# CIS565-Fall-2015/Project3-CUDA-Path-Tracer

Hardware: AMD Instinct MI355X
Metric: Mpaths/sec (paths = pixels x bounces x spp) at 1280x720, 8 bounces (higher is better)
Workload: dtype f32; 1 GPU; scenes/cornell.txt 1280x720, 8 bounces, 64 spp per step x 149 steps; batches_in_flight=3

## Files before the change

### project3-cuda-path-tracer_amd/__init__.py

```python
import ctypes as C
import os

import numpy as np

HERE = os.path.dirname(os.path.abspath(__file__))
LIB_PATH = os.environ.get("PT_AMD_LIB") or os.path.join(HERE, "csrc", "libpt_amd.so")
HOST_LIB_PATH = os.path.join(HERE, "host", "libpt_host.so")

GEOM_DTYPE = np.dtype([
    ("type", "<i4"), ("materialid", "<i4"),
    ("translation", "<f4", 3), ("rotation", "<f4", 3), ("scale", "<f4", 3),
    ("transform", "<f4", 16), ("inverseTransform", "<f4", 16), ("invTranspose", "<f4", 16),
])
MATERIAL_DTYPE = np.dtype([
    ("color", "<f4", 3), ("specularExponent", "<f4"), ("specularColor", "<f4", 3),
    ("hasReflective", "<f4"), ("hasRefractive", "<f4"), ("indexOfRefraction", "<f4"),
    ("emittance", "<f4"),
])
CAMERA_DTYPE = np.dtype([
    ("resolution", "<i4", 2), ("position", "<f4", 3), ("view", "<f4", 3), ("up", "<f4", 3),
    ("fov", "<f4", 2),
])
assert GEOM_DTYPE.itemsize == 236 and MATERIAL_DTYPE.itemsize == 44 and CAMERA_DTYPE.itemsize == 52

# ... 39 lines not shown
    "pt_test_bump_normal", "pt_test_denoise", "pt_test_denoise_var", "pt_test_noise_stats", "pt_test_exp_neg_poly", "pt_test_bounce_form", "pt_test_live_device_buffers",
    "pt_test_renderer_state", "pt_test_scene_plan", "pt_test_temporal", "pt_test_temporal_camera", "pt_test_history",
    "pt_test_display", "pt_test_spatial_variance",
    "pt_test_group_create_virtual", "pt_test_emulated_reduce",
]


class PtOptions(C.Structure):
    _fields_ = [("shard_rank", C.c_int32), ("shard_count", C.c_int32), ("device", C.c_int32),
                ("flags", C.c_int32), ("pipeline_depth", C.c_int32), ("max_batch", C.c_int32),
                ("stream", C.c_void_p), ("accum_dev", C.c_void_p), ("lens_radius", C.c_float), ("focal_distance", C.c_float)]


class PtTestPlanSummary(C.Structure):
    _fields_ = [("state_bits", C.c_uint32)] + [(n, C.c_int32) for n in ("nBinned", "nWalls", "nSphCull", "nSphGroups", "nLocalPad", "firstSkipped", "poolChunks")] + \
               [("ldsBytes", C.c_uint64), ("ldsBytesNext", C.c_uint64)]


class PtMesh(C.Structure):
    _fields_ = [("geom", C.c_int32), ("ntris", C.c_int32), ("tris", C.c_void_p), ("normals", C.c_void_p), ("materials", C.c_void_p)]


class PtTexture(C.Structure):
    _fields_ = [("width", C.c_int32), ("height", C.c_int32), ("rgb", C.c_void_p)]


class PtTexBinding(C.Structure):
    _fields_ = [("geom", C.c_int32), ("texture", C.c_int32), ("ntris", C.c_int32), ("uvs", C.c_void_p)]


class PtBumpBinding(C.Structure):
# ... 1123 lines not shown
```

### project3-cuda-path-tracer_amd/csrc/pt_api.hip

```cpp
#include <hip/hip_runtime.h>

#include <algorithm>
#include <array>
#include <atomic>
#include <condition_variable>
#include <functional>
#include <thread>
#include <cmath>
#include <cstdarg>
#include <cstdio>
#include <cstdlib>
#include <cstring>
#include <deque>
#include <limits>
#include <map>
#include <memory>
#include <string>
#include <utility>
#include <vector>

#include <mutex>

#include "../../include/pt_amd.h"
#include "pt_compaction.h"
// ... 284 lines not shown
    const PathPool out = pool(sl, depth & 1);
    const uint32_t genIn = sl.gen[(depth - 1) & 1];
    if (++R().launchSerial == 0u) ++R().launchSerial;
    const uint32_t genOut = sl.gen[depth & 1] = R().launchSerial;
    hipEvent_t e0 = nullptr, e1 = nullptr;
    if (R().flags & PT_FLAG_KERNEL_TIMING) {
        for (hipEvent_t *e : {&e0, &e1}) {
            if (!R().evFree.empty()) { *e = R().evFree.back(); R().evFree.pop_back(); }
            else HIPCHECK(hipEventCreate(e));
        }
        HIPCHECK(hipEventRecord(e0, sl.stream));
    }
    BounceArgs ba;
    ba.prm = R().prm;
    ba.iter = iter; ba.batch = batch; ba.depth = depth; ba.lastBounce = lastBounce ? 1 : 0; ba.parity = sl.parity;
    ba.genIn = genIn; ba.genOut = genOut;
    ba.in = in; ba.out = out;
    ba.tile.inBase = in.base; ba.tile.inList = in.list; ba.tile.inCap = in.cap;
    ba.tile.genIn = genIn; ba.tile.poolChunks = (uint32_t)R().prm.poolChunks; ba.tile.chunkShift = (uint32_t)R().prm.chunkShift;
    ba.tile.skipNonCandidates = (lastBounce && R().prm.emittersBinned) ? 1u : 0u;
    ba.tile.hot = (lastBounce ? kHotLast : 0u) | (R().prm.allClassified ? kHotAllClassified : 0u) | (contrib ? kHotContrib : 0u) |
                  ((R().prm.directDepth != 0 && depth == R().prm.directDepth && R().prm.nEmit > 0) ? kHotToLight : 0u) |
                  (R().prm.contribLocal ? kHotContribLocal : 0u) | ((R().flags & PT_FLAG_MIXTURE_WEIGHTED) ? kHotMixWeighted : 0u) | ((uint32_t)R().prm.nWalls << 8) | ((uint32_t)R().prm.nSlotWalls << 11) | ((uint32_t)R().prm.nPlaneWalls << 17) |
                  ((uint32_t)R().prm.nBinned << 14) | ((uint32_t)R().prm.nmats << 20);
    const bool lastBits = R().many && !R().mesh && R().prm.sphOMax > 0.0f && R().prm.emittersBinned;
    if (lastBits && nextIsLast) ba.tile.hot |= kHotWritesLastBits;
    if (lastBits && lastBounce && depth > 1) ba.tile.hot |= kHotReadsLastBits;
    ba.ctrl = sl.ctrl.p; ba.ggeoms = R().dgeoms.p; ba.gmats = R().dmats.p; ba.ghit = reinterpret_cast<const float4 *>(R().dGeomHit.p); ba.contrib = contrib; ba.hitMask = sl.hitMask.p;
    ba.sphCull = R().dSphCull.p; ba.classIdx = R().dClassIdx.p;
    ba.rowOff = R().dRowOff.p; ba.rowIdx = R().dRowIdx.p;
// ... 688 lines not shown
        b.geom = bindings[i].geom; b.texture = bindings[i].texture; b.ntris = bindings[i].ntris;
        if (bindings[i].uvs) b.uvs.assign(bindings[i].uvs, bindings[i].uvs + 6 * (size_t)b.ntris);
        R().texBindings.push_back(std::move(b));
    }
    return PT_OK;
}

int pt_init(const PtCamera *cam, const PtGeom *geoms, int ngeoms, const PtMaterial *mats, int nmats, int traceDepth,
            const PtOptions *opts) {
    const PtOptions o = effective_options(opts);
    ScenePlan plan;
    PTCHECK(plan_scene(SceneIn{cam, geoms, ngeoms, mats, nmats, traceDepth, o, R().meshes, R().textures, R().texBindings, R().bumpBindings}, plan));
    const void *kernFirst = nullptr, *kernNext = nullptr;
    PTCHECK(resolve_bounce_kernel(plan, true, &kernFirst));
    PTCHECK(resolve_bounce_kernel(plan, false, &kernNext));
    if (count_devices() < 1) return fail(PT_ERR_NO_GPU, "pt_init: no HIP device (this library has no CPU fallback)");
    register_exit_handler();
    bool keepHistory = R().init && (R().flags & plan.flags & PT_FLAG_TEMPORAL) && R().prm.W == plan.prm.W && R().prm.H == plan.prm.H &&
                       (o.device < 0 || o.device == R().device);
    if (keepHistory && R().committed >= 1 && guide_stack_bytes() > 64 * 1024) keepHistory = false;
    if (keepHistory && R().committed >= 1) {
        const int rc = capture_history();
        if (rc) {
            free_renderer();
            return rc == PT_ERR_INVALID ? fail(PT_ERR_HIP, "pt_init: the capture of the old view failed: %s", std::string(g_err).c_str()) : rc;
        }
    }
    free_renderer(keepHistory);

    State &S = R();
// ... 7 lines not shown
    *S.hostFault = 0u;
    HIPCHECK(hipHostGetDevicePointer((void **)&S.hostFaultDev, S.hostFault, 0));

    if (o.accum_dev) {
        S.image = o.accum_dev;
    } else {
        const size_t n = (S.flags & PT_FLAG_ACCUM_SHARD_ROWS) ? (size_t)(S.nLocal > 0 ? S.nLocal : 1) : (size_t)S.P;
        PTCHECK(S.imageOwn.alloc(n * 3));
        S.image = S.imageOwn.p;
        HIPCHECK(hipMemsetAsync(S.image, 0, n * 3 * sizeof(float), S.stream));
    }
    if (S.flags & PT_FLAG_MOMENTS) PTCHECK(S.moments.alloc_zeroed((size_t)S.P));
    const size_t cpx = S.prm.contribLocal ? (size_t)(S.nLocal > 0 ? S.nLocal : 1) : (size_t)S.P;
    const size_t contribFloats = (size_t)S.maxBatch * cpx * 3, maskWords = (size_t)((S.maxBatch + 31) / 32) * cpx;
    {
        const size_t perSlot = 2 * (S.poolCap * kNumArrays * sizeof(float) + (size_t)kSeg * S.poolChunks * sizeof(unsigned long long)) + sizeof(Ctrl) +
                               contribFloats * sizeof(float) + maskWords * sizeof(uint32_t) + S.meshHitWords * sizeof(unsigned long long);
        const size_t display = (S.flags & PT_FLAG_DISPLAY_FILTER) ? (size_t)S.P * (4 * sizeof(float4) + sizeof(uchar4)) : 0;
        const size_t spatial = (S.flags & PT_FLAG_SPATIAL_VARIANCE) ? (size_t)S.P * sizeof(float) : 0;
        const size_t need = perSlot * (size_t)S.nslots + display + spatial;
        size_t freeB = 0, totalB = 0;
        HIPCHECK(hipMemGetInfo(&freeB, &totalB));
        if (need > freeB)
            return fail(PT_ERR_HIP, "pt_init: %.2f GB of path pools and radiance buffers (max_batch %d x pipeline_depth %d) exceed the %.2f GB of free "
                        "device memory: lower max_batch or pipeline_depth", need / 1e9, S.maxBatch, S.nslots, freeB / 1e9);
    }
    if (S.flags & PT_FLAG_DISPLAY_FILTER) {
        PTCHECK(S.dnPosT.alloc((size_t)S.P));
        PTCHECK(S.dnNrmId.alloc((size_t)S.P));
        for (auto &ping : S.dnPing) PTCHECK(ping.alloc((size_t)S.P));
        PTCHECK(S.dnRgba.alloc((size_t)S.P));
    }
    if (S.flags & PT_FLAG_SPATIAL_VARIANCE) PTCHECK(S.dnCount.alloc((size_t)S.P));
    for (int i = 0; i < S.nslots; ++i) {
        Slot &sl = S.slot[i];
        HIPCHECK(hipStreamCreateWithFlags(&sl.stream, hipStreamNonBlocking));
        for (int b = 0; b < 2; ++b) {
            PTCHECK(sl.pathbuf[b].alloc(S.poolCap * kNumArrays));
            PTCHECK(sl.chunkList[b].alloc_zeroed((size_t)kSeg * S.poolChunks));
        }
        PTCHECK(sl.ctrl.alloc(1));
        PTCHECK(reset_ctrl(sl.ctrl.p, nullptr));
        PTCHECK(sl.contrib.alloc_zeroed(contribFloats));
        PTCHECK(sl.hitMask.alloc_zeroed(maskWords));
        if (S.meshHitWords) PTCHECK(sl.meshHit.alloc(S.meshHitWords));
        HIPCHECK(hipEventCreateWithFlags(&sl.evDone, hipEventDisableTiming));
        HIPCHECK(hipEventCreateWithFlags(&sl.evCommitted, hipEventDisableTiming));
    }

    const auto up = [](auto &buf, const auto &table) { return table.empty() ? (int)PT_OK : buf.upload(table); };
    PTCHECK(up(S.dgeoms, plan.hg));
    PTCHECK(up(S.dmats, plan.hm));
    PTCHECK(up(S.dGeomHit, plan.geomHit));
// ... 479 lines not shown
```

### project3-cuda-path-tracer_amd/csrc/pt_scene_plan.h

```cpp
#pragma once

constexpr int kMaxSlots = 4;
constexpr int kTexSizeMax = 16384;
constexpr long long kTexTexelsMax = 1ll << 28;

struct HostTexture { int w = 0, h = 0; std::vector<float> rgb; };
struct HostTexBinding { int geom = 0, texture = 0, ntris = 0; std::vector<float> uvs; };
struct HostBumpBinding { int geom = 0, texture = 0, ntris = 0; float scale = 0.0f; std::vector<float> uvs; };

struct SceneIn {
    const PtCamera *cam;
    const PtGeom *geoms;
    int ngeoms;
    const PtMaterial *mats;
    int nmats, traceDepth;
    PtOptions o;
    const std::vector<ptm::HostMesh> &meshes;
    const std::vector<HostTexture> &textures;
    const std::vector<HostTexBinding> &texBindings;
    const std::vector<HostBumpBinding> &bumpBindings;
    const ptm::HostMesh *mesh_of(int geom) const {
        for (const ptm::HostMesh &m : meshes)
            if (m.geom == geom) return &m;
        return nullptr;
    }
    bool direct() const { return (o.flags & PT_FLAG_DIRECT_LIGHTING) != 0; }
};

PtOptions effective_options(const PtOptions *opts) {
    PtOptions o;
    memset(&o, 0, sizeof o);
    o.shard_count = 1;
    o.device = -1;
    if (opts) o = *opts;
    return o;
}

inline size_t guideStackBytes(bool mesh, int meshStackNeed) { return mesh ? (size_t)std::max(meshStackNeed, 1) * kBlock * sizeof(uint32_t) : 0; }

struct PlanScalars {
    PtCamera cam;
    KParams prm;
    int P = 0;
    int nLocal = 0;
    int flags = 0;
    int nslots = 0;
    int maxBatch = 1;
    bool grouped = false;
    bool tex = false;
    bool bump = false;
// ... 191 lines not shown
    const int Wp = (Wd + kBlock - 1) / kBlock * kBlock;
    if ((long long)p.rows * Wp >= (1ll << 30)) return fail(PT_ERR_INVALID, "pt_init: frame too large (rows x padded width must stay below 2^30)");
    PTCHECK(checked_magic((uint32_t)Wd, k.magicW, k.shiftW));
    PTCHECK(set_tile_space(k, Wp, p.rows * Wp));
    k.ngeoms = in.ngeoms; k.nmats = in.nmats;
    k.traceDepth = in.traceDepth + (in.direct() ? 1 : 0);
    k.directDepth = in.direct() ? in.traceDepth : 0;
    k.lensRadius = o.lens_radius;
    k.focalDistance = o.focal_distance;
    const H3 vn = hnormalize(H3{in.cam->view.x, in.cam->view.y, in.cam->view.z});
    k.viewN[0] = vn.x; k.viewN[1] = vn.y; k.viewN[2] = vn.z;
    p.dof = o.lens_radius > 0.0f;
    p.plain = !in.direct() && !(o.flags & PT_FLAG_MIXTURE_WEIGHTED) && !env_flag("PT_AMD_NO_PLAIN");
    for (int i = 0; i < in.nmats; ++i)
        if (in.mats[i].hasRefractive > 0.0f || (in.mats[i].hasReflective > 0.0f && in.mats[i].specularExponent > 0.0f)) p.plain = false;
    return PT_OK;
}

void plan_emitters(const SceneIn &in, ScenePlan &p) {
    KParams &k = p.prm;
    k.nEmit = 0;
    for (int i = 0; i < in.ngeoms && k.nEmit < kEmitMax; ++i) {
        float c[3] = {0.0f, 0.0f, 0.0f}, e[3] = {1.0f, 1.0f, 1.0f};
        if (in.geoms[i].type == PT_MESH) {
            const ptm::HostMesh *m = in.mesh_of(i);
            if (!m || m->tris.size() < 9) continue;
            float lo[3] = {m->tris[0], m->tris[1], m->tris[2]}, hi[3] = {lo[0], lo[1], lo[2]};
            for (size_t q = 0; q + 2 < m->tris.size(); q += 3)
                for (int a = 0; a < 3; ++a) {
                    lo[a] = lo[a] < m->tris[q + a] ? lo[a] : m->tris[q + a];
// ... 474 lines not shown
    PTCHECK(check_scene(in));
    PTCHECK(plan_frame(in, p));
    plan_emitters(in, p);
    PTCHECK(plan_pools(in, p));
    PTCHECK(plan_geoms(in, p));
    PTCHECK(plan_camera_cull(in, p));
    plan_bins(in, p);
    plan_walls(in, p);
    PTCHECK(plan_textures(in, p));
    PTCHECK(plan_bump_maps(in, p));
    PTCHECK(plan_swept(in, p));
    plan_hit_records(in, p);
    plan_classes(in, p);
    PTCHECK(plan_camera_list(in, p));
    PTCHECK(plan_walks(in, p));
    return plan_lds(in, p);
}
```

### project3-cuda-path-tracer_amd/csrc/pt_test_api.h

```cpp
#pragma once

int pt_debug_trace_paths(int iter, int bounces, float *origin3, float *dir3, float *color3, int32_t *pixelIndex,
                         int32_t *count) {
    if (!R().init) return fail(PT_ERR_NOT_INIT, "pt_debug_trace_paths before pt_init");
    if (bounces < 0 || bounces > PT_MAX_DEPTH || !count) return fail(PT_ERR_INVALID, "pt_debug_trace_paths: bad argument");
    if (bounces > R().prm.traceDepth) return fail(PT_ERR_INVALID, "pt_debug_trace_paths: bounces > traceDepth");
    int rc = sync_all();
    if (rc) return rc;
    Slot &sl = R().slot[0];
    if (bounces == 0) {
        const int nl = R().nLocal;
        *count = nl;
        if (nl == 0) return PT_OK;
        DevBuf<float> o, d;
        DevBuf<int> px;
        if ((rc = o.alloc((size_t)nl * 3)) || (rc = d.alloc((size_t)nl * 3)) || (rc = px.alloc(nl))) return rc;
        hipLaunchKernelGGL(k_debug_camera_rays, dim3((nl + kBlock - 1) / kBlock), dim3(kBlock), 0, sl.stream, R().prm, iter,
                           o.p, d.p, px.p);
        HIPCHECK(hipGetLastError());
        HIPCHECK(hipStreamSynchronize(sl.stream));
        if (origin3) HIPCHECK(hipMemcpy(origin3, o.p, (size_t)nl * 12, hipMemcpyDeviceToHost));
        if (dir3) HIPCHECK(hipMemcpy(dir3, d.p, (size_t)nl * 12, hipMemcpyDeviceToHost));
        if (pixelIndex) HIPCHECK(hipMemcpy(pixelIndex, px.p, (size_t)nl * 4, hipMemcpyDeviceToHost));
        if (color3)
// ... 19 lines not shown
    const PathPool pb = pool(sl, bounces & 1);
    const uint32_t gen = sl.gen[bounces & 1];
    std::vector<unsigned long long> lists((size_t)kSeg * R().poolChunks);
    HIPCHECK(hipMemcpy(lists.data(), pb.list, lists.size() * sizeof(unsigned long long), hipMemcpyDeviceToHost));
    uint32_t segn[kSeg];
    size_t n = 0;
    for (int sg = 0; sg < kSeg; ++sg) {
        segn[sg] = h.pos[sl.parity][bounces + 1][sg][0];
        n += segn[sg];
    }
    *count = (int32_t)n;
    if (n == 0) return PT_OK;
    const uint32_t chunkPaths = 1u << R().prm.chunkShift;
    std::vector<float> cols[kNumArrays];
    for (int k = 0; k < kNumArrays; ++k) cols[k].resize(n);
    {
        std::vector<float> bufA((size_t)chunkPaths * 4), bufB((size_t)chunkPaths * 4), bufC((size_t)chunkPaths * 3);
        size_t off = 0;
        for (int sg = 0; sg < kSeg; ++sg)
            for (uint32_t done = 0, j = 0; done < segn[sg]; done += chunkPaths, ++j) {
                const uint32_t m = std::min<uint32_t>(chunkPaths, segn[sg] - done);
                const unsigned long long e = lists[(size_t)sg * R().poolChunks + j];
                const uint32_t c = j == 0 ? 1u + (uint32_t)sg : (uint32_t)e;
                if (c == 0 || c >= (uint32_t)R().poolChunks || (j != 0 && (uint32_t)(e >> 32) != gen))
                    return fail(PT_ERR_DEVICE, "pt_debug_trace_paths: corrupt chunk list");
                const size_t first = (size_t)c << R().prm.chunkShift;
                HIPCHECK(hipMemcpy(bufA.data(), pb.arrA(first), (size_t)m * 16, hipMemcpyDeviceToHost));
                HIPCHECK(hipMemcpy(bufB.data(), pb.arrB(first), (size_t)m * 16, hipMemcpyDeviceToHost));
                HIPCHECK(hipMemcpy(bufC.data(), pb.arrC(first), (size_t)m * 12, hipMemcpyDeviceToHost));
                for (uint32_t i = 0; i < m; ++i) {
                    const float *a = &bufA[4 * (size_t)i], *b = &bufB[4 * (size_t)i], *cc = &bufC[3 * (size_t)i];
                    const float v[kNumArrays] = {a[0], a[1], a[2], a[3], b[0], b[1], b[2], b[3], cc[0], cc[1], cc[2]};
                    for (int k = 0; k < kNumArrays; ++k) cols[k][off + i] = v[k];
                }
                off += m;
            }
    }
    const int *pixcol = reinterpret_cast<const int *>(cols[10].data());
    std::vector<size_t> order(n);
    for (size_t i = 0; i < n; ++i) order[i] = i;
    std::sort(order.begin(), order.end(), [&](size_t x, size_t y) { return pixcol[x] < pixcol[y]; });
    float *dst[3] = {origin3, dir3, color3};
    for (size_t i = 0; i < n; ++i) {
        const size_t src = order[i];
        for (int grp = 0; grp < 3; ++grp)
            if (dst[grp])
// ... 31 lines not shown
}

int pt_test_renderer_state(uint32_t *state_bits) {
    if (!state_bits) return fail(PT_ERR_INVALID, "pt_test_renderer_state: bad argument");
    if (!R().init) return fail(PT_ERR_NOT_INIT, "pt_test_renderer_state before pt_init");
    *state_bits = plan_state_bits(R());
    return PT_OK;
}

int pt_test_scene_plan(const PtCamera *cam, const PtGeom *geoms, int ngeoms, const PtMaterial *mats, int nmats, int traceDepth, const PtOptions *opts,
                       PtTestPlanSummary *out) {
    if (!out) return fail(PT_ERR_INVALID, "pt_test_scene_plan: bad argument");
    ScenePlan p;
    PTCHECK(plan_scene(SceneIn{cam, geoms, ngeoms, mats, nmats, traceDepth, effective_options(opts), R().meshes, R().textures, R().texBindings, R().bumpBindings}, p));
    *out = PtTestPlanSummary{plan_state_bits(p), p.prm.nBinned, p.prm.nWalls, p.prm.nSphCull, p.prm.nSphGroups, p.prm.nLocalPad, p.prm.firstSkipped, p.poolChunks,
                             (uint64_t)p.ldsBytes, (uint64_t)p.ldsBytesNext};
    return PT_OK;
}

int64_t pt_test_live_device_buffers(void) { return (int64_t)g_liveDevBufs.load(); }

int pt_test_group_fail_next_reduce(PtGroup *g, int count) {
    if (!g || count < 0) return fail(PT_ERR_INVALID, "pt_test_group_fail_next_reduce: bad argument");
    g->failReduces = count;
    return PT_OK;
}

int pt_test_group_create_virtual(PtGroup **out, int n, const int32_t *vdev, int collective) {
    if (!out || !vdev || n < 1 || n > 64) return fail(PT_ERR_INVALID, "pt_test_group_create_virtual: 1..64 members");
    if (collective != 0 && collective != 1) return fail(PT_ERR_INVALID, "pt_test_group_create_virtual: collective 0 (host gather) or 1 (emulated reduce)");
    if (count_devices() < 1) return fail(PT_ERR_NO_GPU, "pt_test_group_create_virtual: no HIP device");
// ... 1130 lines not shown
```

### project3-cuda-path-tracer_amd/csrc/pt_trace.h

```cpp
#pragma once
#include "../../include/pt_amd.h"
#include <type_traits>

#include "pt_common.h"
#include "pt_device.h"

namespace ptk {
using namespace ptd;

constexpr int kNumArrays = 11;
constexpr int kMaxDepthSlots = PT_MAX_DEPTH + 2;

constexpr int kOct = 8;
constexpr int kCls = 2 * kOct;
constexpr int kSub = 8;
constexpr int kSeg = kCls * kSub;
constexpr int kClsMax = 2 * kCls;
static_assert(kSeg % 64 == 0, "setupTile compares kSeg / 64 prefix entries per lane");
constexpr int kBinMax = 4;
constexpr int kEmitMax = 8;
constexpr int kWallMax = 6;
constexpr int kMinChunkShift = 11;
constexpr int kNanWords = 12;
constexpr int kTicketWords = 4;
constexpr int miscWords(int cls) { return 2 * kWaves * cls + 5 * cls + kSeg + (kSeg + 2) + 2 * PT_MAX_BATCH + 2 + kNanWords + kTicketWords; }
// ... 15 lines not shown
    unsigned long long early[kMaxDepthSlots][kTallyShards][kCtrPad / 2];
    unsigned long long light_hits[kTallyShards][kCtrPad / 2], misses[kTallyShards][kCtrPad / 2];
};
constexpr uint32_t kFaultPoolExhausted = 1u, kFaultReserveTimeout = 2u;
constexpr int kReservePollLimit = 1 << 14;

struct KParams {
    float view[3], up[3], right[3], pos[3];
    float pixLenX, pixLenY, halfW, halfH;
    int   W, H;
    int   shardRank, shardCount;
    int   nLocal;
    int   ngeoms, nmats;
    int   traceDepth;
    int   pixBits;
    int   poolChunks;
    int   chunkShift;
    int   sceneRect[4];
    uint32_t magicW, shiftW, magicN, shiftN;
    int   contribLocal;
    uint32_t magicS, shiftS;
    int   Wp;
    int   nLocalPad;
    int   firstY0;
    int   firstSkipped;
    uint32_t magicWp, shiftWp;
    int   tilesPerRow;
    int   emittersBinned;
    int   nBinned;
    int   binGeom[kBinMax];
// ... 166 lines not shown
    uint32_t hot;
};
constexpr uint32_t kHotLast = 1u, kHotAllClassified = 2u, kHotContrib = 4u, kHotToLight = 8u, kHotContribLocal = 16u;
constexpr uint32_t kHotWritesLastBits = 32u, kHotReadsLastBits = 64u;
constexpr uint32_t kHotMixWeighted = 128u;
__host__ __device__ constexpr uint32_t hotWalls(uint32_t h) { return (h >> 8) & 7u; }
__host__ __device__ constexpr uint32_t hotSlotWalls(uint32_t h) { return (h >> 11) & 7u; }
__host__ __device__ constexpr uint32_t hotPlaneWalls(uint32_t h) { return (h >> 17) & 7u; }
__host__ __device__ constexpr uint32_t hotBinned(uint32_t h) { return (h >> 14) & 7u; }
__host__ __device__ constexpr uint32_t hotMats(uint32_t h) { return h >> 20; }
static_assert(sizeof(TileArgs) == 40, "ten dwords");
struct BounceArgs {
    TileArgs tile;
    KParams prm;
    int iter, batch, depth, lastBounce, parity;
    uint32_t genIn, genOut;
    PathPool in, out;
    Ctrl *ctrl;
    const GeomDev *ggeoms;
    const MaterialDev *gmats;
    const float4 *ghit;
    float *contrib;
    const WallBox *walls;
    const float4 *meshRecs;
    uint32_t *hitMask;
    const SphereCull *sphCull;
    const int *classIdx;
    const int *rowOff;
    const int *rowIdx;
    const uint32_t *camPix;
// ... 222 lines not shown
    uint32_t rowShift = 0;
    constexpr bool kTickets = true;
    const bool ticketed = kTickets && (hotWord & kHotLast) == 0u;
    if (FIRST && !ticketed) {
        const uint32_t tpr = (uint32_t)launder(kargs)->prm.tilesPerRow;
        if (tpr > 1) rowShift = rot = (uint32_t)__builtin_amdgcn_readfirstlane((int)(blockIdx.x % tpr));
    }

    struct TileMeta {
        bool valid;
        uint32_t idx;
        uint32_t cls;
        const float *base;
        uint32_t cap;
    };
    struct PathRegs { F3 org, dir, col; uint32_t pixHash, pk; };
    auto setupTile = [&](uint32_t T, uint32_t tid, TileMeta &m) -> bool {
        const PT_CAS TileArgs &ta = launder(kargs)->tile;
        const uint32_t shift = ta.chunkShift, poolChunks = ta.poolChunks, genIn = ta.genIn, skipNonCand = ta.skipNonCandidates;
        const PT_CAS unsigned long long *const inList = (const PT_CAS unsigned long long *)ta.inList;
        m.base = ta.inBase;
        m.cap = ta.inCap;
        {
            const uint32_t ln = tid & 63u;
            uint32_t cnt = 0u;
#pragma unroll
            for (int q = 0; q < kSeg / 64; ++q) cnt += (uint32_t)__popcll(__ballot(s_segpre[1 + 64 * q + ln] <= T));
            sgIn = cnt;
        }
        probe(26);
        sgIn = (uint32_t)__builtin_amdgcn_readfirstlane((int)sgIn);
// ... 8 lines not shown
        if (j != 0u) {
            const unsigned long long e = j < poolChunks ? inList[(size_t)sgIn * poolChunks + j] : 0ull;
            chunk = (uint32_t)(e >> 32) == genIn ? (uint32_t)e : 0u;
            chunk = chunk < poolChunks ? chunk : 0u;
        }
        m.idx = (chunk << shift) + (local - (j << shift));
        probe(27);
        return true;
    };
    auto loadTile = [&](const TileMeta &m, PathRegs &r) {
        if (m.valid) {
            const char *const src = reinterpret_cast<const char *>(m.base);
            const size_t cap = (size_t)m.cap;
            const float4 a = *reinterpret_cast<const float4 *>(src + 16 * (size_t)m.idx);
            const float4 b = *reinterpret_cast<const float4 *>(src + 16 * cap + 16 * (size_t)m.idx);
            const PathC c = *reinterpret_cast<const PathC *>(src + 32 * cap + 12 * (size_t)m.idx);
            r.org = f3(a.x, a.y, a.z);
            r.dir = f3(a.w, b.x, b.y);
            r.col = f3(b.z, b.w, c.cz);
            r.pixHash = c.pixHash;
            r.pk = c.pk;
        }
    };
    constexpr bool kCamListOk = FIRST && !DOF && !MESH && !MANY;
    const bool camList = kCamListOk && launder(kargs)->camPix != nullptr;
    uint32_t camWord = kCamPad, camItb = 0u, camJ0 = 0u;
    int camSig0 = 0, camSig1 = 0;
    constexpr bool kResolveOk = kCamListOk && !TEX && !BUMP;
    int camFace = -1;
    constexpr bool kWallResolveOk = !FIRST && !MANY && !MESH && !TEX && !BUMP;
    auto requestCam = [&](uint32_t Tq, uint32_t tid) {
        const ArgsPtr A = launder(kargs);
        const uint32_t idx0 = (uint32_t)__builtin_amdgcn_readfirstlane((int)Tq) * kBlock;
        camItb = fastDiv(idx0, A->prm.magicN, A->prm.shiftN);
        camJ0 = idx0 - camItb * (uint32_t)A->prm.nLocalPad;
        camWord = A->camPix[camJ0 + tid];
        const uint32_t wq = (camJ0 >> 6) + (uint32_t)__builtin_amdgcn_readfirstlane((int)(tid >> 6));
        const PT_CAS int *const wr = (const PT_CAS int *)(A->camWave) + 2 * wq;
        camSig0 = wr[0];
        camSig1 = wr[1];
        if (kResolveOk) camFace = ((const PT_CAS int *)(A->camFace))[wq];
    };
    uint32_t T = blockIdx.x - rowShift;
    TileMeta nextMeta = {false, 0u, 0u, nullptr, 0u};
    PathRegs nextRegs = {f3(0, 0, 0), f3(0, 0, 1), f3(0, 0, 0), 0, 0};
    if (!FIRST) {
        while (T < numTiles && !setupTile(T, threadIdx.x, nextMeta)) T += gridDim.x;
        if (T < numTiles) loadTile(nextMeta, nextRegs);
    } else if (camList && T < numTiles) {
        requestCam(T, threadIdx.x);
    }
    __syncthreads();
    uint32_t Tn1 = kTickets ? T + gridDim.x : 0u;
    auto ticketShards = [&]() -> uint32_t { return gridDim.x < (uint32_t)kTicketShards ? gridDim.x : (uint32_t)kTicketShards; };
    while (T < numTiles) {
        uint32_t tid = threadIdx.x;
        asm volatile("" : "+v"(tid));
        T = (uint32_t)__builtin_amdgcn_readfirstlane((int)T);
        probe(14);
        uint32_t Tnext = kTickets ? Tn1 : T + gridDim.x;
// ... 41 lines not shown
                continue;
            }
        } else {
            valid = nextMeta.valid;
            tileCls = nextMeta.cls;
        }

        uint32_t fl = 0u;
        uint32_t smallCandI = 1u;
        uint32_t wallSel = 8u;
        F3 org = anyF3(), dir = anyF3(), col = anyF3();
        int pix = __float_as_int(anyFloat());
        uint32_t pkCur = __float_as_uint(anyFloat());
        auto iterOf = [&]() -> int { return FIRST ? itb : (int)(pkCur >> (uint32_t)launder(kargs)->prm.pixBits); };
        uint32_t pixHash = __float_as_uint(anyFloat());
        if (valid) {
            bool inScene = true;
            if (FIRST) {
                const ArgsPtr A = launder(kargs);
                const PT_CAS KParams &prm = A->prm;
                pix = px + py * prm.W;
                if (!camList) inScene = px >= prm.sceneRect[0] && px <= prm.sceneRect[2] && py >= prm.sceneRect[1] && py <= prm.sceneRect[3];
                if (inScene) {
                    pixHash = utilhash((uint32_t)pix);
                    Rng rng = seedEngine(s_iterHash[PT_MAX_BATCH + itb] ^ pixHash);
                    const float jx = u01(rng);
                    const float jy = u01(rng);
                    const float sx = ((float)px + jx) - prm.halfW;
                    const float sy = ((float)py + jy) - prm.halfH;
                    const float a = prm.pixLenX * sx;
// ... 2 lines not shown
                    const F3 up = f3(prm.up[0], prm.up[1], prm.up[2]);
                    const F3 right = f3(prm.right[0], prm.right[1], prm.right[2]);
                    org = f3(prm.pos[0], prm.pos[1], prm.pos[2]);
                    dir = normalize((view - right * a) - up * b);
                    if (DOF) {
                        const float lr = prm.lensRadius * __builtin_sqrtf(u01(rng));
                        const float phi = u01(rng) * kTwoPi;
                        float s, c;
                        sincosPoly(phi, s, c);
                        const float ft = prm.focalDistance / dot(dir, f3(prm.viewN[0], prm.viewN[1], prm.viewN[2]));
                        const F3 focus = org + dir * ft;
                        org = (org + right * (lr * c)) + up * (lr * s);
                        dir = normalize(focus - org);
                    }
                }
                col = f3(1.0f, 1.0f, 1.0f);
            } else {
                org = cur.org; dir = cur.dir; col = cur.col;
                uint32_t chash = cur.pixHash, cpk = cur.pk;
                if (!MANY) asm volatile("" : "+v"(chash), "+v"(cpk));
                pixHash = chash;
                pkCur = cpk;
            }

            if (FIRST) { if (inScene) probe(8); } else probe(7);
            if (!FIRST) { PT_TALLY_WALL_RESOLVE(0, 1ull); }
            probe(15);
            float tbest = anyFloat();
            int hit = -1;
            F3 P = anyF3(), nsrc = anyF3();
            int outsideI = __float_as_int(anyFloat());
            float2 texBary = make_float2(0.0f, 0.0f);
            uint32_t texUnit = 0u;
            const float dd = dot(dir, dir);
            int nCand = 0;
            float *s_sph = nullptr;
            uint16_t *s_list = nullptr;
// ... 517 lines not shown
                                Pv = mulL(xf, Tv);
                            }
                            const int4 td = A->texDesc[bg.x];
                            float hu, hv;
                            bumpGradient(A->texels, td.x, td.y, td.z, __int_as_float(bg.y), u, v, hu, hv);
                            bumped = tok && bumpNormal(N, Pu, Pv, hu, hv, outside, dir, Ns);
                        }
                    }
                }
                const MaterialDev &M = smats[ghMaterial];
                if (mEmit > 0.0f) {
                    fl = 2u;
                    const ArgsPtr A = launder(kargs);
                    float *const contrib = A->contrib;
                    if (hotNow() & kHotContrib) {
                        const F3 c = (col * mcol) * mEmit;
                        size_t frame = (size_t)A->prm.W * A->prm.H;
                        const uint32_t gpix = FIRST ? (uint32_t)pix : (pkCur & ((1u << (uint32_t)A->prm.pixBits) - 1u));
                        uint32_t cpix = gpix;
                        if (hotNow() & kHotContribLocal) {
                            const uint32_t y = fastDiv(gpix, A->prm.magicW, A->prm.shiftW);
                            const uint32_t lr = fastDiv(y, A->prm.magicS, A->prm.shiftS);
                            cpix = gpix - (y - lr) * (uint32_t)A->prm.W;
                            frame = (size_t)A->prm.nLocal;
                        }
                        const int itq = iterOf();
                        float *dst = contrib + 3 * ((size_t)itq * frame + (size_t)cpix);
                        dst[0] = c.x; dst[1] = c.y; dst[2] = c.z;
                        (void)__hip_atomic_fetch_or(A->hitMask + (size_t)(itq >> 5) * frame + (size_t)cpix, 1u << (itq & 31), __ATOMIC_RELAXED,
                                                    __HIP_MEMORY_SCOPE_AGENT);
                    }
                } else if (!(hotNow() & kHotLast)) {
                    probe(10);
                    Rng rng = seedEngine(s_iterHash[iterOf()] ^ pixHash);
                    const F3 scol = f3(M.specColor[0], M.specColor[1], M.specColor[2]);
                    F3 ndir = dir, norg;
                    bool diffuse = false;
                    bool through = false;
                    if (!PLAIN && mRefr > 0.0f) {
                        const float eta = outside ? M.invIor : M.ior;
                        const float c = dot(Ns, dir);
                        const float k = 1.0f - eta * eta * (1.0f - c * c);
                        const float u = u01(rng);
                        bool doReflect = true;
                        if (k >= 0.0f) {
                            const float r0 = M.r0;
                            const float cosx = outside ? -c : __builtin_sqrtf(k);
                            const float w = 1.0f - cosx;
                            const float w2 = w * w;
                            const float w5 = w2 * w2 * w;
                            const float fres = r0 + (1.0f - r0) * w5;
                            doReflect = u < fres;
                        }
// ... 1 lines not shown
                            ndir = reflect(dir, Ns);
                            norg = P + N * 0.001f;
                            col = col * scol;
                        } else {
                            ndir = refract(dir, Ns, eta);
                            through = true;
                            norg = P - N * 0.001f;
                            col = col * mcol;
                        }
                    } else if (mRefl > 0.0f) {
                        if (!PLAIN && (hotNow() & kHotMixWeighted)) col = col * 2.0f;
                        const float u = u01(rng);
                        if (u < 0.5f) {
                            ndir = reflect(dir, Ns);
                            if (!PLAIN && M.invSpecExp1 > 0.0f) ndir = specularLobeDirection(ndir, Ns, M.invSpecExp1, rng);
                            col = col * scol;
                        } else {
                            diffuse = true;
                        }
                        norg = P + N * 0.001f;
                    } else {
                        diffuse = true;
                        norg = P + N * 0.001f;
                    }
                    bool toLight = false;
                    if (diffuse) {
                        const ArgsPtr A = launder(kargs);
                        toLight = !PLAIN && (hotNow() & kHotToLight) != 0u;
                        if (toLight) {
                            const int ne = A->prm.nEmit;
                            int pick = (int)(u01(rng) * (float)ne);
// ... 10 lines not shown
                            const float uz = u01(rng) - 0.5f;
                            const float *xf = A->ggeoms[e].xf;
                            float m[12];
#pragma unroll
                            for (int q = 0; q < 12; ++q) m[q] = xf[q];
                            const PT_CAS float *bx = &A->prm.emitBox[0][0] + 6 * pick;
                            const F3 target = mulMV(m, f3(bx[0] + ux * bx[3], bx[1] + uy * bx[4], bx[2] + uz * bx[5]), 1.0f);
                            const F3 toward = target - norg;
                            ndir = normalize(toward);
                            float w = dot(Ns, ndir);
                            w = w > 0.0f ? w : 0.0f;
                            float cover = rho2 / dot(toward, toward);
                            cover = cover < 1.0f ? cover : 1.0f;
                            col = (col * mcol) * (w * cover);
                            rng.x = __float_as_uint(anyFloat());
                        } else {
                            col = col * mcol;
                        }
                    }
                    if (diffuse && !toLight) {
                        probe(11);
                        float up, cOver, sOver;
                        hemisphereDraws(rng, up, cOver, sOver);
                        F3 p1, p2;
                        if (isSphere || (BUMP && bumped)) {
                            hemisphereFrame(Ns, p1, p2);
                        } else {
                            p1 = f3(fv[3], fv[4], fv[5]);
                            p2 = f3(fv[6], fv[7], fv[8]);
                        }
                        ndir = hemisphereCombine(Ns, p1, p2, up, cOver, sOver);
                    }
                    org = norg;
                    dir = ndir;
// ... 134 lines not shown
            PT_EXP_EXTRA_BARRIER()
            probe(19);
            if (alive) {
                const ArgsPtr A = launder(kargs);
                uint32_t waveOff = 0u;
#pragma unroll
                for (int w = 0; w < kWaves - 1; ++w) {
                    const uint32_t wq = wv[w * CLS + cls];
                    waveOff += wave > w ? wq : 0u;
                }
                const uint32_t r = waveOff + rank, sp = s_base[CLS + cls];
                const uint32_t slot = r < sp ? s_base[cls] + r : s_base[2 * CLS + cls] + (r - sp);
                char *const dst = reinterpret_cast<char *>(A->out.base);
                const size_t ocap = (size_t)A->out.cap;
                *reinterpret_cast<float4 *>(dst + 16 * (size_t)slot) = make_float4(org.x, org.y, org.z, dir.x);
                *reinterpret_cast<float4 *>(dst + 16 * ocap + 16 * (size_t)slot) = make_float4(dir.y, dir.z, col.x, col.y);
                PathC c;
                c.cz = col.z; c.pixHash = pixHash; c.pk = FIRST ? ((uint32_t)pix | ((uint32_t)itb << (uint32_t)launder(kargs)->prm.pixBits)) : pkCur;
                *reinterpret_cast<PathC *>(dst + 32 * ocap + 12 * (size_t)slot) = c;
            }
            wvSel ^= (uint32_t)(kWaves * CLS);
            if (lane < CLS) s_wave[wvSel + wave * CLS + lane] = 0u;
            __builtin_amdgcn_s_setprio(0);
        } else if (kTickets) {
            Tn1 = Tnext + gridDim.x;
        }
        probe(20);
        T = Tnext;
    }
    censusLeave();
    probe(29);
    const uint32_t waveLight = sLight, waveEarly = sEarly, waveMiss = sMiss + sEarly;
    __syncthreads();
    {
// ... 152 lines not shown
```

Measured before the change: 271,300 Mpaths/s.

## Encode path throughput as packed material history to shrink path pool

For plain scenes (no refraction, glossy, textures, meshes or many objects), each path stores a packed word of per-bounce material codes instead of its colour and pixel hash. The throughput is rebuilt from the material table only when a path hits an emitter, and the pixel hash is recomputed from the pixel index. This cuts the per-path record from 11 to 8 dwords and drops the third array read and write per bounce, at the cost of a short loop over bounces on emitter hits and an extra hash per scatter.

```diff
diff --git a/project3-cuda-path-tracer_amd/__init__.py b/project3-cuda-path-tracer_amd/__init__.py
--- a/project3-cuda-path-tracer_amd/__init__.py
+++ b/project3-cuda-path-tracer_amd/__init__.py
@@ -77,7 +77,7 @@
 
 class PtTestPlanSummary(C.Structure):
     _fields_ = [("state_bits", C.c_uint32)] + [(n, C.c_int32) for n in ("nBinned", "nWalls", "nSphCull", "nSphGroups", "nLocalPad", "firstSkipped", "poolChunks")] + \
-               [("ldsBytes", C.c_uint64), ("ldsBytesNext", C.c_uint64)]
+               [("ldsBytes", C.c_uint64), ("ldsBytesNext", C.c_uint64), ("histBits", C.c_int32), ("reserved", C.c_int32)]
 
 
 class PtMesh(C.Structure):
diff --git a/project3-cuda-path-tracer_amd/csrc/pt_api.hip b/project3-cuda-path-tracer_amd/csrc/pt_api.hip
--- a/project3-cuda-path-tracer_amd/csrc/pt_api.hip
+++ b/project3-cuda-path-tracer_amd/csrc/pt_api.hip
@@ -322,6 +322,7 @@
     BounceArgs ba;
     ba.prm = R().prm;
     ba.iter = iter; ba.batch = batch; ba.depth = depth; ba.lastBounce = lastBounce ? 1 : 0; ba.parity = sl.parity;
+    ba.histShift = R().prm.histBits * (depth - 1);
     ba.genIn = genIn; ba.genOut = genOut;
     ba.in = in; ba.out = out;
     ba.tile.inBase = in.base; ba.tile.inList = in.list; ba.tile.inCap = in.cap;
@@ -1040,6 +1041,8 @@
     const void *kernFirst = nullptr, *kernNext = nullptr;
     PTCHECK(resolve_bounce_kernel(plan, true, &kernFirst));
     PTCHECK(resolve_bounce_kernel(plan, false, &kernNext));
+    if ((plan.prm.histBits != 0) != ((bounce_form(false, plan.dof, plan.many, plan.sweptCubes, plan.mesh, plan.grouped, plan.tex, plan.bump, plan.plain) & kbPlain) != 0))
+        return fail(PT_ERR_INVALID, "pt_init: internal error: history bits %d and the later bounces' form disagree", plan.prm.histBits);
     if (count_devices() < 1) return fail(PT_ERR_NO_GPU, "pt_init: no HIP device (this library has no CPU fallback)");
     register_exit_handler();
     bool keepHistory = R().init && (R().flags & plan.flags & PT_FLAG_TEMPORAL) && R().prm.W == plan.prm.W && R().prm.H == plan.prm.H &&
@@ -1077,7 +1080,7 @@
     const size_t cpx = S.prm.contribLocal ? (size_t)(S.nLocal > 0 ? S.nLocal : 1) : (size_t)S.P;
     const size_t contribFloats = (size_t)S.maxBatch * cpx * 3, maskWords = (size_t)((S.maxBatch + 31) / 32) * cpx;
     {
-        const size_t perSlot = 2 * (S.poolCap * kNumArrays * sizeof(float) + (size_t)kSeg * S.poolChunks * sizeof(unsigned long long)) + sizeof(Ctrl) +
+        const size_t perSlot = 2 * (S.poolCap * poolDwords(S.prm.histBits) * sizeof(float) + (size_t)kSeg * S.poolChunks * sizeof(unsigned long long)) + sizeof(Ctrl) +
                                contribFloats * sizeof(float) + maskWords * sizeof(uint32_t) + S.meshHitWords * sizeof(unsigned long long);
         const size_t display = (S.flags & PT_FLAG_DISPLAY_FILTER) ? (size_t)S.P * (4 * sizeof(float4) + sizeof(uchar4)) : 0;
         const size_t spatial = (S.flags & PT_FLAG_SPATIAL_VARIANCE) ? (size_t)S.P * sizeof(float) : 0;
@@ -1099,7 +1102,7 @@
         Slot &sl = S.slot[i];
         HIPCHECK(hipStreamCreateWithFlags(&sl.stream, hipStreamNonBlocking));
         for (int b = 0; b < 2; ++b) {
-            PTCHECK(sl.pathbuf[b].alloc(S.poolCap * kNumArrays));
+            PTCHECK(sl.pathbuf[b].alloc(S.poolCap * poolDwords(S.prm.histBits)));
             PTCHECK(sl.chunkList[b].alloc_zeroed((size_t)kSeg * S.poolChunks));
         }
         PTCHECK(sl.ctrl.alloc(1));
diff --git a/project3-cuda-path-tracer_amd/csrc/pt_scene_plan.h b/project3-cuda-path-tracer_amd/csrc/pt_scene_plan.h
--- a/project3-cuda-path-tracer_amd/csrc/pt_scene_plan.h
+++ b/project3-cuda-path-tracer_amd/csrc/pt_scene_plan.h
@@ -34,6 +34,12 @@
     o.device = -1;
     if (opts) o = *opts;
     return o;
+}
+
+inline int history_code_bits(int nmats) {
+    int b = 1;
+    while ((1ll << b) < 2ll * nmats) ++b;
+    return b;
 }
 
 inline size_t guideStackBytes(bool mesh, int meshStackNeed) { return mesh ? (size_t)std::max(meshStackNeed, 1) * kBlock * sizeof(uint32_t) : 0; }
@@ -255,6 +261,7 @@
     p.plain = !in.direct() && !(o.flags & PT_FLAG_MIXTURE_WEIGHTED) && !env_flag("PT_AMD_NO_PLAIN");
     for (int i = 0; i < in.nmats; ++i)
         if (in.mats[i].hasRefractive > 0.0f || (in.mats[i].hasReflective > 0.0f && in.mats[i].specularExponent > 0.0f)) p.plain = false;
+    if (history_code_bits(in.nmats) * (k.traceDepth - 1) > 32) p.plain = false;
     return PT_OK;
 }
 
@@ -759,5 +766,6 @@
     plan_classes(in, p);
     PTCHECK(plan_camera_list(in, p));
     PTCHECK(plan_walks(in, p));
+    p.prm.histBits = (p.plain && !p.tex && !p.mesh && !p.many) ? history_code_bits(in.nmats) : 0;
     return plan_lds(in, p);
 }
diff --git a/project3-cuda-path-tracer_amd/csrc/pt_test_api.h b/project3-cuda-path-tracer_amd/csrc/pt_test_api.h
--- a/project3-cuda-path-tracer_amd/csrc/pt_test_api.h
+++ b/project3-cuda-path-tracer_amd/csrc/pt_test_api.h
@@ -57,6 +57,15 @@
     const uint32_t chunkPaths = 1u << R().prm.chunkShift;
     std::vector<float> cols[kNumArrays];
     for (int k = 0; k < kNumArrays; ++k) cols[k].resize(n);
+    const int hb = R().prm.histBits;
+    std::vector<MaterialDev> hmat;
+    if (hb != 0) {
+        if (hb * bounces > 32)
+            return fail(PT_ERR_INVALID, "pt_debug_trace_paths: %d codes of %d bits do not fit a path's history word (the renderer itself scatters %d times)",
+                        bounces, hb, R().prm.traceDepth - 1);
+        hmat.resize((size_t)R().prm.nmats);
+        HIPCHECK(hipMemcpy(hmat.data(), R().dmats.p, hmat.size() * sizeof(MaterialDev), hipMemcpyDeviceToHost));
+    }
     {
         std::vector<float> bufA((size_t)chunkPaths * 4), bufB((size_t)chunkPaths * 4), bufC((size_t)chunkPaths * 3);
         size_t off = 0;
@@ -70,9 +79,23 @@
                 const size_t first = (size_t)c << R().prm.chunkShift;
                 HIPCHECK(hipMemcpy(bufA.data(), pb.arrA(first), (size_t)m * 16, hipMemcpyDeviceToHost));
                 HIPCHECK(hipMemcpy(bufB.data(), pb.arrB(first), (size_t)m * 16, hipMemcpyDeviceToHost));
-                HIPCHECK(hipMemcpy(bufC.data(), pb.arrC(first), (size_t)m * 12, hipMemcpyDeviceToHost));
+                if (hb == 0) HIPCHECK(hipMemcpy(bufC.data(), pb.arrC(first), (size_t)m * 12, hipMemcpyDeviceToHost));
                 for (uint32_t i = 0; i < m; ++i) {
                     const float *a = &bufA[4 * (size_t)i], *b = &bufB[4 * (size_t)i], *cc = &bufC[3 * (size_t)i];
+                    if (hb != 0) {
+                        uint32_t h;
+                        memcpy(&h, &b[2], sizeof h);
+                        float col[3] = {1.0f, 1.0f, 1.0f};
+                        for (int s = 0; s < bounces; ++s, h >>= hb) {
+                            const uint32_t code = h & ((1u << hb) - 1u);
+                            if ((code >> 1) >= (uint32_t)hmat.size()) return fail(PT_ERR_DEVICE, "pt_debug_trace_paths: corrupt history word");
+                            const float *t = (code & 1u) ? hmat[code >> 1].specColor : hmat[code >> 1].color;
+                            for (int q = 0; q < 3; ++q) col[q] = col[q] * t[q];
+                        }
+                        const float v[kNumArrays] = {a[0], a[1], a[2], a[3], b[0], b[1], col[0], col[1], col[2], 0.0f, b[3]};
+                        for (int k = 0; k < kNumArrays; ++k) cols[k][off + i] = v[k];
+                        continue;
+                    }
                     const float v[kNumArrays] = {a[0], a[1], a[2], a[3], b[0], b[1], b[2], b[3], cc[0], cc[1], cc[2]};
                     for (int k = 0; k < kNumArrays; ++k) cols[k][off + i] = v[k];
                 }
@@ -134,7 +157,7 @@
     ScenePlan p;
     PTCHECK(plan_scene(SceneIn{cam, geoms, ngeoms, mats, nmats, traceDepth, effective_options(opts), R().meshes, R().textures, R().texBindings, R().bumpBindings}, p));
     *out = PtTestPlanSummary{plan_state_bits(p), p.prm.nBinned, p.prm.nWalls, p.prm.nSphCull, p.prm.nSphGroups, p.prm.nLocalPad, p.prm.firstSkipped, p.poolChunks,
-                             (uint64_t)p.ldsBytes, (uint64_t)p.ldsBytesNext};
+                             (uint64_t)p.ldsBytes, (uint64_t)p.ldsBytesNext, p.prm.histBits, 0};
     return PT_OK;
 }
 
diff --git a/project3-cuda-path-tracer_amd/csrc/pt_trace.h b/project3-cuda-path-tracer_amd/csrc/pt_trace.h
--- a/project3-cuda-path-tracer_amd/csrc/pt_trace.h
+++ b/project3-cuda-path-tracer_amd/csrc/pt_trace.h
@@ -9,6 +9,8 @@
 using namespace ptd;
 
 constexpr int kNumArrays = 11;
+constexpr int kNumArraysHist = 8;
+__host__ __device__ constexpr int poolDwords(int histBits) { return histBits ? kNumArraysHist : kNumArrays; }
 constexpr int kMaxDepthSlots = PT_MAX_DEPTH + 2;
 
 constexpr int kOct = 8;
@@ -54,6 +56,7 @@
     int   ngeoms, nmats;
     int   traceDepth;
     int   pixBits;
+    int   histBits;
     int   poolChunks;
     int   chunkShift;
     int   sceneRect[4];
@@ -250,6 +253,7 @@
     TileArgs tile;
     KParams prm;
     int iter, batch, depth, lastBounce, parity;
+    int histShift;
     uint32_t genIn, genOut;
     PathPool in, out;
     Ctrl *ctrl;
@@ -502,7 +506,9 @@
         const float *base;
         uint32_t cap;
     };
-    struct PathRegs { F3 org, dir, col; uint32_t pixHash, pk; };
+    constexpr bool HIST = PLAIN;
+    constexpr bool kFeedsHist = FIRST && DOF && !MANY && !MESH && !TEX;
+    struct PathRegs { F3 org, dir, col; uint32_t pixHash, pk, hist; };
     auto setupTile = [&](uint32_t T, uint32_t tid, TileMeta &m) -> bool {
         const PT_CAS TileArgs &ta = launder(kargs)->tile;
         const uint32_t shift = ta.chunkShift, poolChunks = ta.poolChunks, genIn = ta.genIn, skipNonCand = ta.skipNonCandidates;
@@ -541,12 +547,19 @@
             const size_t cap = (size_t)m.cap;
             const float4 a = *reinterpret_cast<const float4 *>(src + 16 * (size_t)m.idx);
             const float4 b = *reinterpret_cast<const float4 *>(src + 16 * cap + 16 * (size_t)m.idx);
-            const PathC c = *reinterpret_cast<const PathC *>(src + 32 * cap + 12 * (size_t)m.idx);
-            r.org = f3(a.x, a.y, a.z);
-            r.dir = f3(a.w, b.x, b.y);
-            r.col = f3(b.z, b.w, c.cz);
-            r.pixHash = c.pixHash;
-            r.pk = c.pk;
+            if (HIST) {
+                r.org = f3(a.x, a.y, a.z);
+                r.dir = f3(a.w, b.x, b.y);
+                r.hist = __float_as_uint(b.z);
+                r.pk = __float_as_uint(b.w);
+            } else {
+                const PathC c = *reinterpret_cast<const PathC *>(src + 32 * cap + 12 * (size_t)m.idx);
+                r.org = f3(a.x, a.y, a.z);
+                r.dir = f3(a.w, b.x, b.y);
+                r.col = f3(b.z, b.w, c.cz);
+                r.pixHash = c.pixHash;
+                r.pk = c.pk;
+            }
         }
     };
     constexpr bool kCamListOk = FIRST && !DOF && !MESH && !MANY;
@@ -570,7 +583,7 @@
     };
     uint32_t T = blockIdx.x - rowShift;
     TileMeta nextMeta = {false, 0u, 0u, nullptr, 0u};
-    PathRegs nextRegs = {f3(0, 0, 0), f3(0, 0, 1), f3(0, 0, 0), 0, 0};
+    PathRegs nextRegs = {f3(0, 0, 0), f3(0, 0, 1), f3(0, 0, 0), 0, 0, 0};
     if (!FIRST) {
         while (T < numTiles && !setupTile(T, threadIdx.x, nextMeta)) T += gridDim.x;
         if (T < numTiles) loadTile(nextMeta, nextRegs);
@@ -642,6 +655,8 @@
         uint32_t pkCur = __float_as_uint(anyFloat());
         auto iterOf = [&]() -> int { return FIRST ? itb : (int)(pkCur >> (uint32_t)launder(kargs)->prm.pixBits); };
         uint32_t pixHash = __float_as_uint(anyFloat());
+        uint32_t hist = 0u;
+        if (HIST && !FIRST) hist = __float_as_uint(anyFloat());
         if (valid) {
             bool inScene = true;
             if (FIRST) {
@@ -674,13 +689,21 @@
                         dir = normalize(focus - org);
                     }
                 }
-                col = f3(1.0f, 1.0f, 1.0f);
+                if (!HIST) col = f3(1.0f, 1.0f, 1.0f);
             } else {
-                org = cur.org; dir = cur.dir; col = cur.col;
-                uint32_t chash = cur.pixHash, cpk = cur.pk;
-                if (!MANY) asm volatile("" : "+v"(chash), "+v"(cpk));
-                pixHash = chash;
-                pkCur = cpk;
+                org = cur.org; dir = cur.dir;
+                if (!HIST) col = cur.col;
+                if (HIST) {
+                    uint32_t chist = cur.hist, cpk = cur.pk;
+                    asm volatile("" : "+v"(chist), "+v"(cpk));
+                    hist = chist;
+                    pkCur = cpk;
+                } else {
+                    uint32_t chash = cur.pixHash, cpk = cur.pk;
+                    if (!MANY) asm volatile("" : "+v"(chash), "+v"(cpk));
+                    pixHash = chash;
+                    pkCur = cpk;
+                }
             }
 
             if (FIRST) { if (inScene) probe(8); } else probe(7);
@@ -1228,6 +1251,21 @@
                     const ArgsPtr A = launder(kargs);
                     float *const contrib = A->contrib;
                     if (hotNow() & kHotContrib) {
+                        if (HIST) {
+                            col = f3(1.0f, 1.0f, 1.0f);
+                            if (!FIRST) {
+                                const uint32_t hb = (uint32_t)A->prm.histBits, steps = (uint32_t)A->depth - 1u;
+                                const uint32_t mask = (1u << hb) - 1u;
+                                uint32_t h = hist;
+                                for (uint32_t s = 0; s < steps; ++s) {
+                                    const uint32_t code = h & mask;
+                                    h >>= hb;
+                                    const MaterialDev &Mk = smats[code >> 1];
+                                    const float *const t = (code & 1u) ? Mk.specColor : Mk.color;
+                                    col = col * f3(t[0], t[1], t[2]);
+                                }
+                            }
+                        }
                         const F3 c = (col * mcol) * mEmit;
                         size_t frame = (size_t)A->prm.W * A->prm.H;
                         const uint32_t gpix = FIRST ? (uint32_t)pix : (pkCur & ((1u << (uint32_t)A->prm.pixBits) - 1u));
@@ -1246,11 +1284,13 @@
                     }
                 } else if (!(hotNow() & kHotLast)) {
                     probe(10);
+                    if (HIST && !FIRST) pixHash = utilhash(pkCur & ((1u << (uint32_t)launder(kargs)->prm.pixBits) - 1u));
                     Rng rng = seedEngine(s_iterHash[iterOf()] ^ pixHash);
                     const F3 scol = f3(M.specColor[0], M.specColor[1], M.specColor[2]);
                     F3 ndir = dir, norg;
                     bool diffuse = false;
                     bool through = false;
+                    uint32_t hcode = 0u;
                     if (!PLAIN && mRefr > 0.0f) {
                         const float eta = outside ? M.invIor : M.ior;
                         const float c = dot(Ns, dir);
@@ -1282,7 +1322,8 @@
                         if (u < 0.5f) {
                             ndir = reflect(dir, Ns);
                             if (!PLAIN && M.invSpecExp1 > 0.0f) ndir = specularLobeDirection(ndir, Ns, M.invSpecExp1, rng);
-                            col = col * scol;
+                            if (HIST || kFeedsHist) hcode = 1u;
+                            if (!HIST) col = col * scol;
                         } else {
                             diffuse = true;
                         }
@@ -1323,10 +1364,12 @@
                             cover = cover < 1.0f ? cover : 1.0f;
                             col = (col * mcol) * (w * cover);
                             rng.x = __float_as_uint(anyFloat());
-                        } else {
+                        } else if (!HIST) {
                             col = col * mcol;
                         }
                     }
+                    if (HIST) hist |= (2u * (uint32_t)ghMaterial + hcode) << (uint32_t)launder(kargs)->histShift;
+                    else if (kFeedsHist) hist = 2u * (uint32_t)ghMaterial + hcode;
                     if (diffuse && !toLight) {
                         probe(11);
                         float up, cOver, sOver;
@@ -1491,10 +1534,15 @@
                 char *const dst = reinterpret_cast<char *>(A->out.base);
                 const size_t ocap = (size_t)A->out.cap;
                 *reinterpret_cast<float4 *>(dst + 16 * (size_t)slot) = make_float4(org.x, org.y, org.z, dir.x);
-                *reinterpret_cast<float4 *>(dst + 16 * ocap + 16 * (size_t)slot) = make_float4(dir.y, dir.z, col.x, col.y);
-                PathC c;
-                c.cz = col.z; c.pixHash = pixHash; c.pk = FIRST ? ((uint32_t)pix | ((uint32_t)itb << (uint32_t)launder(kargs)->prm.pixBits)) : pkCur;
-                *reinterpret_cast<PathC *>(dst + 32 * ocap + 12 * (size_t)slot) = c;
+                if (HIST || (kFeedsHist && A->prm.histBits != 0)) {
+                    const uint32_t pk = FIRST ? ((uint32_t)pix | ((uint32_t)itb << (uint32_t)launder(kargs)->prm.pixBits)) : pkCur;
+                    *reinterpret_cast<float4 *>(dst + 16 * ocap + 16 * (size_t)slot) = make_float4(dir.y, dir.z, __uint_as_float(hist), __uint_as_float(pk));
+                } else {
+                    *reinterpret_cast<float4 *>(dst + 16 * ocap + 16 * (size_t)slot) = make_float4(dir.y, dir.z, col.x, col.y);
+                    PathC c;
+                    c.cz = col.z; c.pixHash = pixHash; c.pk = FIRST ? ((uint32_t)pix | ((uint32_t)itb << (uint32_t)launder(kargs)->prm.pixBits)) : pkCur;
+                    *reinterpret_cast<PathC *>(dst + 32 * ocap + 12 * (size_t)slot) = c;
+                }
             }
             wvSel ^= (uint32_t)(kWaves * CLS);
             if (lane < CLS) s_wave[wvSel + wave * CLS + lane] = 0u;
```

Result: faster. 313,000 Mpaths/s (median of 6 runs) (+15.3%).
